# FrozenWolf-Cyber/Indic-CL-ASR

Measured on AMD Instinct MI355X. Metric: utterances/sec (15 s @16 kHz) Conformer-M RNNT-CTC+EWC train step, higher is better.
Workload: dtype bf16; 1 GPU; BASELINE configs[1]: Conformer-medium (d=256, 16L, H=640) hybrid RNNT-CTC + EWC, bs=32/GPU x 15 s, bf16 projections, freeze_encoder_till=12, 22x257 heads, fused_batch_size=4; global_batch=32, parallelism=dp1

## Files before the change

indic_cl_asr_amd/csrc/lstm.hip:

```cpp
#include <hip/hip_bf16.h>

#include <stdlib.h>

#include "ia_common.h"

namespace {

typedef __bf16 bf8 __attribute__((ext_vector_type(8)));
typedef float f4 __attribute__((ext_vector_type(4)));
typedef __attribute__((address_space(1))) unsigned gu32;

constexpr int LS_HB = 16;
constexpr int LS_THREADS = 256;
constexpr int LS_MAXB = 32;
constexpr unsigned LS_SPIN_LIMIT = 1u << 22;
constexpr int LS_STICKY_WORD = 32;

__device__ __forceinline__ float sigmoidf_(float x) { return 1.f / (1.f + __expf(-x)); }

__device__ __forceinline__ void grid_arrive(unsigned* counter) {
    asm volatile("s_waitcnt vmcnt(0)" ::: "memory");
    __syncthreads();
    if (threadIdx.x == 0) __hip_atomic_fetch_add(counter, 1u, __ATOMIC_RELAXED, __HIP_MEMORY_SCOPE_AGENT);
}
__device__ __forceinline__ void ls_store_pair(__bf16* p, float v, bool live) {
    union { __bf16 h; unsigned short u; } me;
    me.h = (__bf16)v;
    const unsigned mine = me.u;
    const unsigned other = (unsigned)__shfl_down((int)mine, 1, 64);
    if (live && !(threadIdx.x & 1))
        __hip_atomic_store((gu32*)(unsigned*)(void*)p, mine | (other << 16), __ATOMIC_RELAXED, __HIP_MEMORY_SCOPE_AGENT);
}
__device__ __forceinline__ void grid_wait(unsigned* counter, unsigned target, unsigned* status, unsigned spin_limit) {
    if (threadIdx.x == 0) {
        unsigned spins = 0;
        while (__hip_atomic_load(counter, __ATOMIC_RELAXED, __HIP_MEMORY_SCOPE_AGENT) < target) {
            __builtin_amdgcn_s_sleep(2);
            if (++spins > spin_limit) {
                __hip_atomic_store(status + 1, 1u, __ATOMIC_RELAXED, __HIP_MEMORY_SCOPE_AGENT);
                __hip_atomic_store(status + LS_STICKY_WORD, 1u, __ATOMIC_RELAXED, __HIP_MEMORY_SCOPE_AGENT);
                break;
            }
        }
        __builtin_amdgcn_fence(__ATOMIC_ACQUIRE, "agent");
        asm volatile("s_waitcnt vmcnt(0)" ::: "memory");
    }
    __syncthreads();
}

__global__ __launch_bounds__(LS_THREADS, 1) void lstm_fwd_kernel(
    const float* __restrict__ Gx,
    const __bf16* __restrict__ Whh,
    float* __restrict__ Hout,
    float* __restrict__ gates,
    float* __restrict__ Cs,
    __bf16* hx,
    unsigned* sync,
    int U, int B, int H, unsigned spin_limit) {
    extern __shared__ __attribute__((aligned(16))) unsigned char smem[];
    const int wrow = H * 2 + 16;
    unsigned char* sW = smem;
    unsigned char* sH = sW + 64 * wrow;
    float* sG = reinterpret_cast<float*>(sH + LS_MAXB * wrow);
    const int tid = threadIdx.x, lane = tid & 63, wave = tid >> 6, c = lane & 15, q4 = lane >> 4;
    const int j = blockIdx.x, nb = gridDim.x, u0 = j * LS_HB;
    const int nrt = (B + 15) / 16;
    for (int i = tid; i < 64 * (H / 8); i += LS_THREADS) {
        const int r = i / (H / 8), v = i - r * (H / 8);
        const int gate = r >> 4, ul = r & 15;
        *reinterpret_cast<uint4*>(sW + r * wrow + v * 16) =
            *reinterpret_cast<const uint4*>(Whh + (size_t)(gate * H + u0 + ul) * H + v * 8);
    }
    for (int i = tid; i < (LS_MAXB - B) * (H / 8); i += LS_THREADS) {
        const int r = B + i / (H / 8), v = i % (H / 8);
        *reinterpret_cast<uint4*>(sH + r * wrow + v * 16) = make_uint4(0, 0, 0, 0);
    }
    constexpr int EPT = (LS_MAXB * LS_HB) / LS_THREADS;
    float cst[EPT];
#pragma unroll
    for (int k = 0; k < EPT; ++k) cst[k] = 0.f;
    __syncthreads();
    float gxp[EPT][4];
#define LS_FETCH_GX(t_)                                                                                   \
    _Pragma("unroll") for (int k = 0; k < EPT; ++k) {                                                     \
        const int e_ = tid + LS_THREADS * k, b_ = e_ >> 4, ul_ = e_ & 15;                                 \
        const size_t gx_ = ((size_t)(t_) * B + (b_ < B ? b_ : B - 1)) * (4 * H) + u0 + ul_;              \
        gxp[k][0] = Gx[gx_]; gxp[k][1] = Gx[gx_ + H]; gxp[k][2] = Gx[gx_ + 2 * H]; gxp[k][3] = Gx[gx_ + 3 * H]; \
    }
    LS_FETCH_GX(0);
    for (int t = 0; t < U; ++t) {
        constexpr int NRT = LS_MAXB / 16;
        f4 acc[NRT];
#pragma unroll
        for (int rt = 0; rt < NRT; ++rt) acc[rt] = (f4){0.f, 0.f, 0.f, 0.f};
        if (t > 0) {
            grid_wait(sync, (unsigned)(nb * t), sync, spin_limit);
            const __bf16* hsrc = hx + (size_t)((t - 1) & 1) * B * H;
            for (int i = tid; i < B * (H / 8); i += LS_THREADS) {
                const int r = i / (H / 8), v = i - r * (H / 8);
                *reinterpret_cast<uint4*>(sH + r * wrow + v * 16) = *reinterpret_cast<const uint4*>(hsrc + (size_t)r * H + v * 8);
            }
            __syncthreads();
            const unsigned char* wb = sW + (wave * 16 + c) * wrow + q4 * 16;
            for (int ks = 0; ks < H / 32; ++ks) {
                const bf8 wf = *reinterpret_cast<const bf8*>(wb + ks * 64);
#pragma unroll
                for (int rt = 0; rt < NRT; ++rt)
                    if (rt < nrt) {
                        const bf8 hf = *reinterpret_cast<const bf8*>(sH + (rt * 16 + c) * wrow + q4 * 16 + ks * 64);
                        acc[rt] = __builtin_amdgcn_mfma_f32_16x16x32_bf16(hf, wf, acc[rt], 0, 0, 0);
                    }
            }
        }
#pragma unroll
        for (int rt = 0; rt < NRT; ++rt)
            if (rt < nrt)
#pragma unroll
                for (int r = 0; r < 4; ++r) sG[(wave * LS_MAXB + rt * 16 + q4 * 4 + r) * 16 + c] = acc[rt][r];
        __syncthreads();
        __bf16* hdst = hx + (size_t)(t & 1) * B * H;
        float kg[EPT][4], kh[EPT];
#pragma unroll
        for (int k = 0; k < EPT; ++k) {
            const int e = tid + LS_THREADS * k, b = e >> 4, ul = e & 15;
            if (b < B) {
                const float gi = sigmoidf_(sG[(0 * LS_MAXB + b) * 16 + ul] + gxp[k][0]);
                const float gf = sigmoidf_(sG[(1 * LS_MAXB + b) * 16 + ul] + gxp[k][1]);
                const float gg = tanhf(sG[(2 * LS_MAXB + b) * 16 + ul] + gxp[k][2]);
                const float go = sigmoidf_(sG[(3 * LS_MAXB + b) * 16 + ul] + gxp[k][3]);
                cst[k] = gf * cst[k] + gi * gg;
                const float h = go * tanhf(cst[k]);
                kg[k][0] = gi; kg[k][1] = gf; kg[k][2] = gg; kg[k][3] = go; kh[k] = h;
            } else {
                kh[k] = 0.f;
            }
            ls_store_pair(hdst + (size_t)(b < B ? b : 0) * H + u0 + ul, kh[k], b < B);
        }
        if (t + 1 < U) grid_arrive(sync);
#pragma unroll
        for (int k = 0; k < EPT; ++k) {
            const int e = tid + LS_THREADS * k, b = e >> 4, ul = e & 15;
            if (b < B) {
                const size_t gx = ((size_t)t * B + b) * (4 * H) + u0 + ul;
                const size_t ho = ((size_t)t * B + b) * H + u0 + ul;
                Hout[ho] = kh[k];
                if (gates) {
                    gates[gx] = kg[k][0]; gates[gx + H] = kg[k][1]; gates[gx + 2 * H] = kg[k][2]; gates[gx + 3 * H] = kg[k][3];
                    Cs[ho] = cst[k];
                }
            }
        }
        if (t + 1 < U) LS_FETCH_GX(t + 1);
    }
#undef LS_FETCH_GX
}

__global__ __launch_bounds__(LS_THREADS, 1) void lstm_bwd_kernel(
    const float* __restrict__ dHout,
    const float* __restrict__ gates,
    const float* __restrict__ Cs,
    const __bf16* __restrict__ WhhT,
    float* __restrict__ dG,
    __bf16* dgx,
    unsigned* sync, int U, int B, int H, unsigned spin_limit) {
    extern __shared__ __attribute__((aligned(16))) unsigned char smem[];
    const int H4 = 4 * H;
    const int wrow = H4 * 2 + 16;
    unsigned char* sW = smem;
    float* sP = reinterpret_cast<float*>(sW + LS_HB * wrow);
    const int tid = threadIdx.x, lane = tid & 63, wave = tid >> 6, c = lane & 15, q4 = lane >> 4;
    const int j = blockIdx.x, nb = gridDim.x, u0 = j * LS_HB;
    const int nrt = (B + 15) / 16;
    for (int i = tid; i < LS_HB * (H4 / 8); i += LS_THREADS) {
        const int r = i / (H4 / 8), v = i - r * (H4 / 8);
        *reinterpret_cast<uint4*>(sW + r * wrow + v * 16) = *reinterpret_cast<const uint4*>(WhhT + (size_t)(u0 + r) * H4 + v * 8);
    }
    constexpr int EPT = (LS_MAXB * LS_HB) / LS_THREADS;
    float dcc[EPT];
#pragma unroll
    for (int k = 0; k < EPT; ++k) dcc[k] = 0.f;
    __syncthreads();
    const int ksteps = H4 / 32, kper = (ksteps + 3) / 4;
    float pv[EPT][7];
#define LS_FETCH_SAVED(t_)                                                                                \
    _Pragma("unroll") for (int k = 0; k < EPT; ++k) {                                                     \
        const int e_ = tid + LS_THREADS * k, b_ = e_ >> 4, ul_ = e_ & 15;                                 \
        const int bc_ = b_ < B ? b_ : B - 1;                                                              \
        const size_t ho_ = ((size_t)(t_) * B + bc_) * H + u0 + ul_;                                       \
        const size_t gx_ = ((size_t)(t_) * B + bc_) * H4 + u0 + ul_;                                      \
        pv[k][0] = dHout[ho_]; pv[k][1] = gates[gx_]; pv[k][2] = gates[gx_ + H]; pv[k][3] = gates[gx_ + 2 * H]; \
        pv[k][4] = gates[gx_ + 3 * H]; pv[k][5] = Cs[ho_]; pv[k][6] = ((t_) > 0) ? Cs[ho_ - (size_t)B * H] : 0.f; \
    }
    LS_FETCH_SAVED(U - 1);
    for (int t = U - 1; t >= 0; --t) {
        const int phase = U - 1 - t;
        constexpr int NRT = LS_MAXB / 16;
        f4 acc[NRT];
#pragma unroll
        for (int rt = 0; rt < NRT; ++rt) acc[rt] = (f4){0.f, 0.f, 0.f, 0.f};
        if (t < U - 1) {
            grid_wait(sync, (unsigned)(nb * phase), sync, spin_limit);
            const __bf16* src = dgx + (size_t)((phase - 1) & 1) * B * H4;
            const int k0 = wave * kper, k1 = (k0 + kper < ksteps) ? (k0 + kper) : ksteps;
            for (int ks = k0; ks < k1; ++ks) {
                const bf8 wf = *reinterpret_cast<const bf8*>(sW + c * wrow + ks * 64 + q4 * 16);
#pragma unroll
                for (int rt = 0; rt < NRT; ++rt)
                    if (rt < nrt) {
                        int brow = rt * 16 + c;
                        brow = brow < B ? brow : B - 1;
                        const bf8 df = *reinterpret_cast<const bf8*>(src + (size_t)brow * H4 + ks * 32 + q4 * 8);
                        acc[rt] = __builtin_amdgcn_mfma_f32_16x16x32_bf16(df, wf, acc[rt], 0, 0, 0);
                    }
            }
        }
#pragma unroll
        for (int rt = 0; rt < NRT; ++rt)
            if (rt < nrt)
#pragma unroll
                for (int r = 0; r < 4; ++r) sP[(wave * LS_MAXB + rt * 16 + q4 * 4 + r) * 16 + c] = acc[rt][r];
        __syncthreads();
        __bf16* dst = dgx + (size_t)(phase & 1) * B * H4;
        float kd[EPT][4];
#pragma unroll
        for (int k = 0; k < EPT; ++k) {
            const int e = tid + LS_THREADS * k, b = e >> 4, ul = e & 15;
            if (b < B) {
                const float dhrec = sP[(0 * LS_MAXB + b) * 16 + ul] + sP[(1 * LS_MAXB + b) * 16 + ul] +
                                    sP[(2 * LS_MAXB + b) * 16 + ul] + sP[(3 * LS_MAXB + b) * 16 + ul];
                const float dh = pv[k][0] + dhrec;
                const float gi = pv[k][1], gf = pv[k][2], gg = pv[k][3], go = pv[k][4];
                const float ct = pv[k][5], cprev = pv[k][6];
                const float tc = tanhf(ct);
                const float dct = dh * go * (1.f - tc * tc) + dcc[k];
                const float di = dct * gg * gi * (1.f - gi);
                const float dfg = dct * cprev * gf * (1.f - gf);
                const float dgg = dct * gi * (1.f - gg * gg);
                const float dout = dh * tc * go * (1.f - go);
                dcc[k] = dct * gf;
                kd[k][0] = di; kd[k][1] = dfg; kd[k][2] = dgg; kd[k][3] = dout;
            } else {
                kd[k][0] = kd[k][1] = kd[k][2] = kd[k][3] = 0.f;
            }
            {
                __bf16* xo = dst + (size_t)(b < B ? b : 0) * H4 + u0 + ul;
#pragma unroll
                for (int gte = 0; gte < 4; ++gte) ls_store_pair(xo + (size_t)gte * H, kd[k][gte], b < B);
            }
        }
        if (t > 0) grid_arrive(sync);
#pragma unroll
        for (int k = 0; k < EPT; ++k) {
            const int e = tid + LS_THREADS * k, b = e >> 4, ul = e & 15;
            if (b < B) {
                const size_t gx = ((size_t)t * B + b) * H4 + u0 + ul;
                dG[gx] = kd[k][0]; dG[gx + H] = kd[k][1]; dG[gx + 2 * H] = kd[k][2]; dG[gx + 3 * H] = kd[k][3];
            }
        }
        if (t > 0) LS_FETCH_SAVED(t - 1);
        __syncthreads();
    }
#undef LS_FETCH_SAVED
}

}

extern "C" size_t ia_lstm_scratch_bytes(int B, int H) {
    if (B <= 0 || H <= 0) return 0;
    return 256 + ia_align_up((size_t)2 * B * 4 * H * sizeof(__bf16), 256);
}

static unsigned lstm_spin_limit() {
    const char* e = getenv("IA_LSTM_SPIN_LIMIT");
    if (e && *e) { const long v = atol(e); if (v >= 0) return (unsigned)v; }
    return LS_SPIN_LIMIT;
}

extern "C" int ia_lstm_lds_bytes(int H, int backward) {
    if (H <= 0) return 0;
    return backward ? (int)((size_t)LS_HB * (4 * H * 2 + 16) + 4 * LS_MAXB * 16 * sizeof(float))
                    : (int)((size_t)(64 + LS_MAXB) * (H * 2 + 16) + 4 * LS_MAXB * 16 * sizeof(float));
}

static int lstm_check(int U, int B, int H) {
    if (U <= 0 || B <= 0 || H <= 0) return IA_INVALID_VALUE;
    if (B > LS_MAXB || H % 32 != 0 || H % LS_HB != 0 || H / LS_HB > 256) return IA_UNSUPPORTED;
    return IA_OK;
}

extern "C" int ia_lstm_forward(const float* Gx, const void* Whh_bf16, float* Hout, float* gates, float* Cs, int U, int B,
                               int H, void* scratch, size_t scratch_bytes, ia_stream_t stream) {
    if (!Gx || !Whh_bf16 || !Hout || !scratch || (gates && !Cs)) return IA_INVALID_VALUE;
    const int rc = lstm_check(U, B, H);
    if (rc != IA_OK) return rc;
    if (scratch_bytes < ia_lstm_scratch_bytes(B, H) || !ia_is_aligned(scratch, 256) || !ia_is_aligned(Whh_bf16, 16))
        return IA_INVALID_VALUE;
    hipStream_t st = (hipStream_t)stream;
    if (hipMemsetAsync(scratch, 0, 128, st) != hipSuccess) return IA_LAUNCH_FAILED;
    const size_t lds = (size_t)(64 + LS_MAXB) * (H * 2 + 16) + 4 * LS_MAXB * 16 * sizeof(float);
    if (lds > 160 * 1024) return IA_UNSUPPORTED;
    IA_SET_MAX_LDS_ONCE((lstm_fwd_kernel), (int)lds);
    hipLaunchKernelGGL(lstm_fwd_kernel, dim3(H / LS_HB), dim3(LS_THREADS), lds, st, Gx, (const __bf16*)Whh_bf16, Hout, gates, Cs,
                       (__bf16*)((char*)scratch + 256), (unsigned*)scratch, U, B, H, lstm_spin_limit());
    IA_RETURN_IF_LAUNCH_FAILED();
    return IA_OK;
}

extern "C" int ia_lstm_backward(const float* dHout, const float* gates, const float* Cs, const void* WhhT_bf16, float* dG,
                                int U, int B, int H, void* scratch, size_t scratch_bytes, ia_stream_t stream) {
    if (!dHout || !gates || !Cs || !WhhT_bf16 || !dG || !scratch) return IA_INVALID_VALUE;
    const int rc = lstm_check(U, B, H);
    if (rc != IA_OK) return rc;
    if (scratch_bytes < ia_lstm_scratch_bytes(B, H) || !ia_is_aligned(scratch, 256) || !ia_is_aligned(WhhT_bf16, 16))
        return IA_INVALID_VALUE;
    hipStream_t st = (hipStream_t)stream;
    if (hipMemsetAsync(scratch, 0, 128, st) != hipSuccess) return IA_LAUNCH_FAILED;
    const size_t lds = (size_t)LS_HB * (4 * H * 2 + 16) + 4 * LS_MAXB * 16 * sizeof(float);
    if (lds > 160 * 1024) return IA_UNSUPPORTED;
    IA_SET_MAX_LDS_ONCE((lstm_bwd_kernel), (int)lds);
    hipLaunchKernelGGL(lstm_bwd_kernel, dim3(H / LS_HB), dim3(LS_THREADS), lds, st, dHout, gates, Cs, (const __bf16*)WhhT_bf16, dG,
                       (__bf16*)((char*)scratch + 256), (unsigned*)scratch, U, B, H, lstm_spin_limit());
    IA_RETURN_IF_LAUNCH_FAILED();
    return IA_OK;
}
```

indic_cl_asr_amd/csrc/dwconv.hip:

```cpp
#include <hip/hip_bf16.h>

#include <cstdint>
#include <cstdlib>

#include "ia_common.h"
#include "indicasr.h"
#include "partials.h"

namespace {

constexpr int DW_TT = 16;
constexpr int DW_TB = 4 * DW_TT;

template <int KMAX>
__device__ __forceinline__ void load_taps(float (&wt)[KMAX], const float* __restrict__ w, int c, int ksz, int flip) {
    const int off = (KMAX - 1) / 2 - (ksz - 1) / 2;
#pragma unroll
    for (int jj = 0; jj < KMAX; ++jj) {
        const int j = jj - off;
        wt[jj] = (j >= 0 && j < ksz) ? w[c * ksz + (flip ? ksz - 1 - j : j)] : 0.f;
    }
}

template <int KMAX, int GLU>
// ... 129 lines not shown
    if (wv == 0 && cok) {
        float* row = part + (size_t)blockIdx.x * (KMAX + 1) * d;
#pragma unroll
        for (int jj = 0; jj < KMAX; ++jj)
            row[(size_t)jj * d + c] = (acc[jj] + red[0][jj][lane]) + (red[1][jj][lane] + red[2][jj][lane]);
        row[(size_t)KMAX * d + c] = (sb + red[0][KMAX][lane]) + (red[1][KMAX][lane] + red[2][KMAX][lane]);
    }
}

__global__ __launch_bounds__(256) void dwconv_wgrad_finish_kernel(const float* __restrict__ part, int G, int d, int kmax, int ksz,
                                                                  float* __restrict__ dw, float* __restrict__ db) {
    __shared__ float red[8][32];
    const int o = threadIdx.x & 31, sl = threadIdx.x >> 5;
    const int idx = blockIdx.x * 32 + o, total = (kmax + 1) * d;
    float a0 = 0.f, a1 = 0.f;
    if (idx < total) {
        int g = sl;
        for (; g + 8 < G; g += 16) { a0 += part[(size_t)g * total + idx]; a1 += part[(size_t)(g + 8) * total + idx]; }
        for (; g < G; g += 8) a0 += part[(size_t)g * total + idx];
    }
    red[sl][o] = a0 + a1;
    __syncthreads();
    if (sl != 0 || idx >= total) return;
    const float s = ((red[0][o] + red[1][o]) + (red[2][o] + red[3][o])) + ((red[4][o] + red[5][o]) + (red[6][o] + red[7][o]));
    const int jj = idx / d, c = idx - jj * d;
    if (jj == kmax) {
        if (db) db[c] = s;
    } else {
        const int j = jj - ((kmax - 1) / 2 - (ksz - 1) / 2);
        if (j >= 0 && j < ksz) dw[c * ksz + j] = s;
    }
}

inline int kmax_for(int ksz) { return ksz <= 9 ? 9 : (ksz <= 15 ? 15 : 31); }

inline int wgrad_splits(int B, int T, int d) {
    const int cg = (d + 63) / 64;
    int ns = (768 + B * cg - 1) / (B * cg);
    const int cap = (T + DW_TB - 1) / DW_TB;
    if (ns > cap) ns = cap;
    return ns < 1 ? 1 : ns;
}

inline bool dw_shape_ok(int d, int ksz) { return d > 0 && d <= 4096 && ksz >= 1 && ksz <= 31 && (ksz & 1) == 1; }

}

extern "C" int64_t ia_dwconv_scratch_elems(int B, int T, int d, int ksz) {
    if (B <= 0 || T <= 0 || !dw_shape_ok(d, ksz)) return 0;
    const int64_t fwd = (int64_t)B * ((T + DW_TB - 1) / DW_TB) * 2 * d;
    const int64_t wg = (int64_t)B * wgrad_splits(B, T, d) * (kmax_for(ksz) + 1) * d;
    return fwd > wg ? fwd : wg;
}

extern "C" int ia_glu_dwconv(const void* x2, const int64_t* lens, int B, int T, int d, int ksz, const float* w,
                             const float* bias, float* z, float* bn_sum, float* bn_sumsq, float* scratch,
                             ia_stream_t stream) {
    if (!x2 || !lens || !w || !bias || !z || !bn_sum || !bn_sumsq || !scratch || B <= 0 || T <= 0) return IA_INVALID_VALUE;
    if (!dw_shape_ok(d, ksz)) return IA_UNSUPPORTED;
    hipStream_t st = (hipStream_t)stream;
    const dim3 grid(B * ((T + DW_TB - 1) / DW_TB), (d + 63) / 64), blk(256);
#define IA_DWF(K) hipLaunchKernelGGL((dwconv_fwd_kernel<K, 1>), grid, blk, 0, st, x2, lens, B, T, d, ksz, w, bias, 0, z, scratch, (long long*)nullptr)
    switch (kmax_for(ksz)) {
        case 9: IA_DWF(9); break;
        case 15: IA_DWF(15); break;
        default: IA_DWF(31); break;
    }
#undef IA_DWF
    IA_RETURN_IF_LAUNCH_FAILED();
    ia_partials_finish(scratch, (int)grid.x, 2 * d, d, bn_sum, bn_sumsq, st);
    IA_RETURN_IF_LAUNCH_FAILED();
    return IA_OK;
}

extern "C" int ia_glu_dwconv_fixed(const void* x2, const int64_t* lens, int B, int T, int d, int ksz, const float* w,
                                   const float* bias, float* z, long long* bn_sums_fixed, ia_stream_t stream) {
    if (!x2 || !lens || !w || !bias || !z || !bn_sums_fixed || B <= 0 || T <= 0) return IA_INVALID_VALUE;
    if (!dw_shape_ok(d, ksz)) return IA_UNSUPPORTED;
    hipStream_t st = (hipStream_t)stream;
    const dim3 grid(B * ((T + DW_TB - 1) / DW_TB), (d + 63) / 64), blk(256);
#define IA_DWF(K) hipLaunchKernelGGL((dwconv_fwd_kernel<K, 1>), grid, blk, 0, st, x2, lens, B, T, d, ksz, w, bias, 0, z, (float*)nullptr, bn_sums_fixed)
    switch (kmax_for(ksz)) {
        case 9: IA_DWF(9); break;
        case 15: IA_DWF(15); break;
        default: IA_DWF(31); break;
    }
#undef IA_DWF
    IA_RETURN_IF_LAUNCH_FAILED();
    return IA_OK;
}

extern "C" int ia_dwconv_gated_fixed(const void* g, const int64_t* lens, int B, int T, int d, int ksz, const float* w,
                                     const float* bias, float* z, long long* bn_sums_fixed, ia_stream_t stream) {
    if (!g || !lens || !w || !bias || !z || !bn_sums_fixed || B <= 0 || T <= 0) return IA_INVALID_VALUE;
    if (!dw_shape_ok(d, ksz)) return IA_UNSUPPORTED;
    hipStream_t st = (hipStream_t)stream;
    const dim3 grid(B * ((T + DW_TB - 1) / DW_TB), (d + 63) / 64), blk(256);
#define IA_DWF(K) hipLaunchKernelGGL((dwconv_fwd_kernel<K, 2>), grid, blk, 0, st, g, lens, B, T, d, ksz, w, bias, 0, z, (float*)nullptr, bn_sums_fixed)
    switch (kmax_for(ksz)) {
        case 9: IA_DWF(9); break;
        case 15: IA_DWF(15); break;
        default: IA_DWF(31); break;
    }
#undef IA_DWF
    IA_RETURN_IF_LAUNCH_FAILED();
    return IA_OK;
}

extern "C" int ia_dwconv_time(const float* x, int B, int T, int d, int ksz, const float* w, const float* bias, int flip,
                              float* y, ia_stream_t stream) {
    if (!x || !w || !y || B <= 0 || T <= 0) return IA_INVALID_VALUE;
    if (!dw_shape_ok(d, ksz)) return IA_UNSUPPORTED;
    hipStream_t st = (hipStream_t)stream;
    const dim3 grid(B * ((T + DW_TB - 1) / DW_TB), (d + 63) / 64), blk(256);
#define IA_DWF(K) hipLaunchKernelGGL((dwconv_fwd_kernel<K, 0>), grid, blk, 0, st, (const void*)x, (const int64_t*)nullptr, B, T, d, ksz, w, bias, flip, y, (float*)nullptr, (long long*)nullptr)
    switch (kmax_for(ksz)) {
        case 9: IA_DWF(9); break;
        case 15: IA_DWF(15); break;
        default: IA_DWF(31); break;
    }
#undef IA_DWF
    IA_RETURN_IF_LAUNCH_FAILED();
    return IA_OK;
}

extern "C" int ia_dwconv_time_wgrad(const float* x, const float* dy, int B, int T, int d, int ksz, float* dw, float* db,
                                    float* scratch, ia_stream_t stream) {
    if (!x || !dy || !dw || !scratch || B <= 0 || T <= 0) return IA_INVALID_VALUE;
    if (!dw_shape_ok(d, ksz)) return IA_UNSUPPORTED;
    hipStream_t st = (hipStream_t)stream;
    const int ns = wgrad_splits(B, T, d), kmax = kmax_for(ksz);
    const dim3 grid(B * ns, (d + 63) / 64), blk(256);
#define IA_DWG(K) hipLaunchKernelGGL((dwconv_wgrad_kernel<K, false>), grid, blk, 0, st, x, dy, B, T, d, ns, scratch, (const __bf16*)nullptr, (const int64_t*)nullptr)
    switch (kmax) {
        case 9: IA_DWG(9); break;
        case 15: IA_DWG(15); break;
        default: IA_DWG(31); break;
    }
#undef IA_DWG
    IA_RETURN_IF_LAUNCH_FAILED();
    hipLaunchKernelGGL(dwconv_wgrad_finish_kernel, dim3(((kmax + 1) * d + 31) / 32), dim3(256), 0, st, scratch, (int)grid.x, d,
                       kmax, ksz, dw, db);
    IA_RETURN_IF_LAUNCH_FAILED();
    return IA_OK;
}

extern "C" int ia_dwconv_glu_bwd(const float* dz, const void* c2, const int64_t* lens, int B, int T, int d, int ksz, const float* w,
                                 void* dc2, ia_stream_t stream) {
    if (!dz || !c2 || !lens || !w || !dc2 || B <= 0 || T <= 0) return IA_INVALID_VALUE;
    if (!dw_shape_ok(d, ksz)) return IA_UNSUPPORTED;
    hipStream_t st = (hipStream_t)stream;
    const dim3 grid(B * ((T + DW_TB - 1) / DW_TB), (d + 63) / 64), blk(256);
#define IA_DWF(K) hipLaunchKernelGGL((dwconv_fwd_kernel<K, 3>), grid, blk, 0, st, (const void*)dz, lens, B, T, d, ksz, w, (const float*)nullptr, 1, (float*)nullptr, (float*)nullptr, (long long*)nullptr, (const __bf16*)c2, (__bf16*)dc2)
    switch (kmax_for(ksz)) {
        case 9: IA_DWF(9); break;
        case 15: IA_DWF(15); break;
        default: IA_DWF(31); break;
    }
#undef IA_DWF
    IA_RETURN_IF_LAUNCH_FAILED();
    return IA_OK;
}

extern "C" int ia_dwconv_glu_wgrad(const void* c2, const int64_t* lens, const float* dy, int B, int T, int d, int ksz, float* dw,
                                   float* db, float* scratch, ia_stream_t stream) {
    if (!c2 || !lens || !dy || !dw || !scratch || B <= 0 || T <= 0) return IA_INVALID_VALUE;
    if (!dw_shape_ok(d, ksz)) return IA_UNSUPPORTED;
    hipStream_t st = (hipStream_t)stream;
    const int ns = wgrad_splits(B, T, d), kmax = kmax_for(ksz);
    const dim3 grid(B * ns, (d + 63) / 64), blk(256);
#define IA_DWG(K) hipLaunchKernelGGL((dwconv_wgrad_kernel<K, true>), grid, blk, 0, st, (const float*)nullptr, dy, B, T, d, ns, scratch, (const __bf16*)c2, lens)
    switch (kmax) {
        case 9: IA_DWG(9); break;
        case 15: IA_DWG(15); break;
        default: IA_DWG(31); break;
    }
#undef IA_DWG
    IA_RETURN_IF_LAUNCH_FAILED();
    hipLaunchKernelGGL(dwconv_wgrad_finish_kernel, dim3(((kmax + 1) * d + 31) / 32), dim3(256), 0, st, scratch, (int)grid.x, d,
                       kmax, ksz, dw, db);
    IA_RETURN_IF_LAUNCH_FAILED();
    return IA_OK;
}
```

Before: 3779 utterances/s.

## Keep LSTM recurrent weights resident in registers instead of LDS for H=640/320

Adds templated LSTM forward and backward kernels that preload each wave's slice of the recurrent weight matrix into bf8 registers once. Each timestep's MFMA loop then reads only h or dgates from LDS or global memory, not the weights, so per-step LDS traffic drops and the LDS footprint shrinks. The K loops are fully unrolled with a compile-time step count, and the FMA ordering is pinned explicitly. The cost is much higher register pressure, and the launch bounds now ask for two blocks per CU. The path is limited to H of 640 or 320 and can be turned off with an environment variable.

Measured after the change: 3788 utterances/s, median of 5. Within noise of the previous version (+0.2%).

```diff
diff --git a/indic_cl_asr_amd/csrc/lstm.hip b/indic_cl_asr_amd/csrc/lstm.hip
--- a/indic_cl_asr_amd/csrc/lstm.hip
+++ b/indic_cl_asr_amd/csrc/lstm.hip
@@ -17,6 +17,7 @@
 constexpr int LS_STICKY_WORD = 32;
 
 __device__ __forceinline__ float sigmoidf_(float x) { return 1.f / (1.f + __expf(-x)); }
+
 
 __device__ __forceinline__ void grid_arrive(unsigned* counter) {
     asm volatile("s_waitcnt vmcnt(0)" ::: "memory");
@@ -48,7 +49,37 @@
     __syncthreads();
 }
 
-__global__ __launch_bounds__(LS_THREADS, 1) void lstm_fwd_kernel(
+__host__ __device__ constexpr size_t ls_fwd_lds(int H, bool wreg) {
+    return (size_t)((wreg ? 0 : 64) + LS_MAXB) * (H * 2 + 16) + 4 * LS_MAXB * LS_HB * sizeof(float);
+}
+__host__ __device__ constexpr size_t ls_bwd_lds(int H, bool wreg) {
+    return (wreg ? 0 : (size_t)LS_HB * (4 * H * 2 + 16)) + 4 * LS_MAXB * LS_HB * sizeof(float);
+}
+
+template <int KS, int NR>
+__device__ __forceinline__ void ls_fwd_dot(f4 (&acc)[LS_MAXB / 16], const bf8 (&wf)[KS], const unsigned char* hb, int wrow) {
+#pragma unroll
+    for (int ks = 0; ks < KS; ++ks)
+#pragma unroll
+        for (int rt = 0; rt < NR; ++rt) {
+            const bf8 hf = *reinterpret_cast<const bf8*>(hb + rt * 16 * wrow + ks * 64);
+            acc[rt] = __builtin_amdgcn_mfma_f32_16x16x32_bf16(hf, wf[ks], acc[rt], 0, 0, 0);
+        }
+}
+template <int KS, int NR>
+__device__ __forceinline__ void ls_bwd_dot(f4 (&acc)[LS_MAXB / 16], const bf8 (&wf)[KS], const __bf16* const (&drow)[LS_MAXB / 16],
+                                           int kofs) {
+#pragma unroll
+    for (int i = 0; i < KS; ++i)
+#pragma unroll
+        for (int rt = 0; rt < NR; ++rt) {
+            const bf8 df = *reinterpret_cast<const bf8*>(drow[rt] + kofs + i * 32);
+            acc[rt] = __builtin_amdgcn_mfma_f32_16x16x32_bf16(df, wf[i], acc[rt], 0, 0, 0);
+        }
+}
+
+template <int KS>
+__global__ __launch_bounds__(LS_THREADS, KS ? 2 : 1) void lstm_fwd_kernel(
     const float* __restrict__ Gx,
     const __bf16* __restrict__ Whh,
     float* __restrict__ Hout,
@@ -56,20 +87,28 @@
     float* __restrict__ Cs,
     __bf16* hx,
     unsigned* sync,
-    int U, int B, int H, unsigned spin_limit) {
+    int U, int B, int Hrt, unsigned spin_limit) {
     extern __shared__ __attribute__((aligned(16))) unsigned char smem[];
+    const int H = KS ? KS * 32 : Hrt;
     const int wrow = H * 2 + 16;
     unsigned char* sW = smem;
-    unsigned char* sH = sW + 64 * wrow;
+    unsigned char* sH = sW + (KS ? 0 : 64) * wrow;
     float* sG = reinterpret_cast<float*>(sH + LS_MAXB * wrow);
     const int tid = threadIdx.x, lane = tid & 63, wave = tid >> 6, c = lane & 15, q4 = lane >> 4;
     const int j = blockIdx.x, nb = gridDim.x, u0 = j * LS_HB;
     const int nrt = (B + 15) / 16;
-    for (int i = tid; i < 64 * (H / 8); i += LS_THREADS) {
-        const int r = i / (H / 8), v = i - r * (H / 8);
-        const int gate = r >> 4, ul = r & 15;
-        *reinterpret_cast<uint4*>(sW + r * wrow + v * 16) =
-            *reinterpret_cast<const uint4*>(Whh + (size_t)(gate * H + u0 + ul) * H + v * 8);
+    bf8 wf[KS ? KS : 1];
+    if constexpr (KS > 0) {
+        const __bf16* wg = Whh + (size_t)(wave * H + u0 + c) * H + q4 * 8;
+#pragma unroll
+        for (int ks = 0; ks < KS; ++ks) wf[ks] = *reinterpret_cast<const bf8*>(wg + ks * 32);
+    } else {
+        for (int i = tid; i < 64 * (H / 8); i += LS_THREADS) {
+            const int r = i / (H / 8), v = i - r * (H / 8);
+            const int gate = r >> 4, ul = r & 15;
+            *reinterpret_cast<uint4*>(sW + r * wrow + v * 16) =
+                *reinterpret_cast<const uint4*>(Whh + (size_t)(gate * H + u0 + ul) * H + v * 8);
+        }
     }
     for (int i = tid; i < (LS_MAXB - B) * (H / 8); i += LS_THREADS) {
         const int r = B + i / (H / 8), v = i % (H / 8);
@@ -101,15 +140,21 @@
                 *reinterpret_cast<uint4*>(sH + r * wrow + v * 16) = *reinterpret_cast<const uint4*>(hsrc + (size_t)r * H + v * 8);
             }
             __syncthreads();
-            const unsigned char* wb = sW + (wave * 16 + c) * wrow + q4 * 16;
-            for (int ks = 0; ks < H / 32; ++ks) {
-                const bf8 wf = *reinterpret_cast<const bf8*>(wb + ks * 64);
-#pragma unroll
-                for (int rt = 0; rt < NRT; ++rt)
-                    if (rt < nrt) {
-                        const bf8 hf = *reinterpret_cast<const bf8*>(sH + (rt * 16 + c) * wrow + q4 * 16 + ks * 64);
-                        acc[rt] = __builtin_amdgcn_mfma_f32_16x16x32_bf16(hf, wf, acc[rt], 0, 0, 0);
-                    }
+            const unsigned char* hb = sH + c * wrow + q4 * 16;
+            if constexpr (KS > 0) {
+                if (nrt == NRT) ls_fwd_dot<KS, NRT>(acc, wf, hb, wrow);
+                else ls_fwd_dot<KS, 1>(acc, wf, hb, wrow);
+            } else {
+                const unsigned char* wb = sW + (wave * 16 + c) * wrow + q4 * 16;
+                for (int ks = 0; ks < H / 32; ++ks) {
+                    const bf8 wl = *reinterpret_cast<const bf8*>(wb + ks * 64);
+#pragma unroll
+                    for (int rt = 0; rt < NRT; ++rt)
+                        if (rt < nrt) {
+                            const bf8 hf = *reinterpret_cast<const bf8*>(hb + rt * 16 * wrow + ks * 64);
+                            acc[rt] = __builtin_amdgcn_mfma_f32_16x16x32_bf16(hf, wl, acc[rt], 0, 0, 0);
+                        }
+                }
             }
         }
 #pragma unroll
@@ -122,13 +167,14 @@
         float kg[EPT][4], kh[EPT];
 #pragma unroll
         for (int k = 0; k < EPT; ++k) {
+#pragma clang fp contract(off)
             const int e = tid + LS_THREADS * k, b = e >> 4, ul = e & 15;
             if (b < B) {
                 const float gi = sigmoidf_(sG[(0 * LS_MAXB + b) * 16 + ul] + gxp[k][0]);
                 const float gf = sigmoidf_(sG[(1 * LS_MAXB + b) * 16 + ul] + gxp[k][1]);
                 const float gg = tanhf(sG[(2 * LS_MAXB + b) * 16 + ul] + gxp[k][2]);
                 const float go = sigmoidf_(sG[(3 * LS_MAXB + b) * 16 + ul] + gxp[k][3]);
-                cst[k] = gf * cst[k] + gi * gg;
+                cst[k] = __builtin_fmaf(gi, gg, gf * cst[k]);
                 const float h = go * tanhf(cst[k]);
                 kg[k][0] = gi; kg[k][1] = gf; kg[k][2] = gg; kg[k][3] = go; kh[k] = h;
             } else {
@@ -155,32 +201,42 @@
 #undef LS_FETCH_GX
 }
 
-__global__ __launch_bounds__(LS_THREADS, 1) void lstm_bwd_kernel(
+template <int KS>
+__global__ __launch_bounds__(LS_THREADS, KS ? 2 : 1) void lstm_bwd_kernel(
     const float* __restrict__ dHout,
     const float* __restrict__ gates,
     const float* __restrict__ Cs,
     const __bf16* __restrict__ WhhT,
     float* __restrict__ dG,
     __bf16* dgx,
-    unsigned* sync, int U, int B, int H, unsigned spin_limit) {
+    unsigned* sync, int U, int B, int Hrt, unsigned spin_limit) {
     extern __shared__ __attribute__((aligned(16))) unsigned char smem[];
+    const int H = KS ? KS * 32 : Hrt;
     const int H4 = 4 * H;
     const int wrow = H4 * 2 + 16;
     unsigned char* sW = smem;
-    float* sP = reinterpret_cast<float*>(sW + LS_HB * wrow);
+    float* sP = reinterpret_cast<float*>(sW + (KS ? 0 : LS_HB) * wrow);
     const int tid = threadIdx.x, lane = tid & 63, wave = tid >> 6, c = lane & 15, q4 = lane >> 4;
     const int j = blockIdx.x, nb = gridDim.x, u0 = j * LS_HB;
     const int nrt = (B + 15) / 16;
-    for (int i = tid; i < LS_HB * (H4 / 8); i += LS_THREADS) {
-        const int r = i / (H4 / 8), v = i - r * (H4 / 8);
-        *reinterpret_cast<uint4*>(sW + r * wrow + v * 16) = *reinterpret_cast<const uint4*>(WhhT + (size_t)(u0 + r) * H4 + v * 8);
+    const int ksteps = H4 / 32, kper = (ksteps + 3) / 4;
+    const int k0 = wave * kper, k1 = (k0 + kper < ksteps) ? (k0 + kper) : ksteps;
+    bf8 wf[KS ? KS : 1];
+    if constexpr (KS > 0) {
+        const __bf16* wg = WhhT + (size_t)(u0 + c) * H4 + k0 * 32 + q4 * 8;
+#pragma unroll
+        for (int i = 0; i < KS; ++i) wf[i] = *reinterpret_cast<const bf8*>(wg + i * 32);
+    } else {
+        for (int i = tid; i < LS_HB * (H4 / 8); i += LS_THREADS) {
+            const int r = i / (H4 / 8), v = i - r * (H4 / 8);
+            *reinterpret_cast<uint4*>(sW + r * wrow + v * 16) = *reinterpret_cast<const uint4*>(WhhT + (size_t)(u0 + r) * H4 + v * 8);
+        }
     }
     constexpr int EPT = (LS_MAXB * LS_HB) / LS_THREADS;
     float dcc[EPT];
 #pragma unroll
     for (int k = 0; k < EPT; ++k) dcc[k] = 0.f;
     __syncthreads();
-    const int ksteps = H4 / 32, kper = (ksteps + 3) / 4;
     float pv[EPT][7];
 #define LS_FETCH_SAVED(t_)                                                                                \
     _Pragma("unroll") for (int k = 0; k < EPT; ++k) {                                                     \
@@ -201,17 +257,25 @@
         if (t < U - 1) {
             grid_wait(sync, (unsigned)(nb * phase), sync, spin_limit);
             const __bf16* src = dgx + (size_t)((phase - 1) & 1) * B * H4;
-            const int k0 = wave * kper, k1 = (k0 + kper < ksteps) ? (k0 + kper) : ksteps;
-            for (int ks = k0; ks < k1; ++ks) {
-                const bf8 wf = *reinterpret_cast<const bf8*>(sW + c * wrow + ks * 64 + q4 * 16);
-#pragma unroll
-                for (int rt = 0; rt < NRT; ++rt)
-                    if (rt < nrt) {
-                        int brow = rt * 16 + c;
-                        brow = brow < B ? brow : B - 1;
-                        const bf8 df = *reinterpret_cast<const bf8*>(src + (size_t)brow * H4 + ks * 32 + q4 * 8);
-                        acc[rt] = __builtin_amdgcn_mfma_f32_16x16x32_bf16(df, wf, acc[rt], 0, 0, 0);
-                    }
+            const __bf16* drow[NRT];
+#pragma unroll
+            for (int rt = 0; rt < NRT; ++rt) {
+                const int brow = rt * 16 + c;
+                drow[rt] = src + (size_t)(brow < B ? brow : B - 1) * H4 + q4 * 8;
+            }
+            if constexpr (KS > 0) {
+                if (nrt == NRT) ls_bwd_dot<KS, NRT>(acc, wf, drow, k0 * 32);
+                else ls_bwd_dot<KS, 1>(acc, wf, drow, k0 * 32);
+            } else {
+                for (int ks = k0; ks < k1; ++ks) {
+                    const bf8 wl = *reinterpret_cast<const bf8*>(sW + c * wrow + ks * 64 + q4 * 16);
+#pragma unroll
+                    for (int rt = 0; rt < NRT; ++rt)
+                        if (rt < nrt) {
+                            const bf8 df = *reinterpret_cast<const bf8*>(drow[rt] + ks * 32);
+                            acc[rt] = __builtin_amdgcn_mfma_f32_16x16x32_bf16(df, wl, acc[rt], 0, 0, 0);
+                        }
+                }
             }
         }
 #pragma unroll
@@ -224,6 +288,7 @@
         float kd[EPT][4];
 #pragma unroll
         for (int k = 0; k < EPT; ++k) {
+#pragma clang fp contract(off)
             const int e = tid + LS_THREADS * k, b = e >> 4, ul = e & 15;
             if (b < B) {
                 const float dhrec = sP[(0 * LS_MAXB + b) * 16 + ul] + sP[(1 * LS_MAXB + b) * 16 + ul] +
@@ -232,7 +297,7 @@
                 const float gi = pv[k][1], gf = pv[k][2], gg = pv[k][3], go = pv[k][4];
                 const float ct = pv[k][5], cprev = pv[k][6];
                 const float tc = tanhf(ct);
-                const float dct = dh * go * (1.f - tc * tc) + dcc[k];
+                const float dct = __builtin_fmaf(dh * go, 1.f - tc * tc, dcc[k]);
                 const float di = dct * gg * gi * (1.f - gi);
                 const float dfg = dct * cprev * gf * (1.f - gf);
                 const float dgg = dct * gi * (1.f - gg * gg);
@@ -276,15 +341,46 @@
     return LS_SPIN_LIMIT;
 }
 
+static int lstm_wreg_ksteps(int H) {
+    if (H != 640 && H != 320) return 0;
+    const char* e = getenv("IA_LSTM_WREG");
+    if (e && e[0] == '0' && !e[1]) return 0;
+    return H / 32;
+}
+
 extern "C" int ia_lstm_lds_bytes(int H, int backward) {
     if (H <= 0) return 0;
-    return backward ? (int)((size_t)LS_HB * (4 * H * 2 + 16) + 4 * LS_MAXB * 16 * sizeof(float))
-                    : (int)((size_t)(64 + LS_MAXB) * (H * 2 + 16) + 4 * LS_MAXB * 16 * sizeof(float));
+    const bool wreg = lstm_wreg_ksteps(H) > 0;
+    return (int)(backward ? ls_bwd_lds(H, wreg) : ls_fwd_lds(H, wreg));
 }
 
 static int lstm_check(int U, int B, int H) {
     if (U <= 0 || B <= 0 || H <= 0) return IA_INVALID_VALUE;
     if (B > LS_MAXB || H % 32 != 0 || H % LS_HB != 0 || H / LS_HB > 256) return IA_UNSUPPORTED;
+    return IA_OK;
+}
+
+template <int KS>
+static int lstm_launch_fwd(const float* Gx, const __bf16* Whh, float* Hout, float* gates, float* Cs, int U, int B, int H,
+                           void* scratch, hipStream_t st) {
+    const size_t lds = ls_fwd_lds(H, KS > 0);
+    if (lds > 160 * 1024) return IA_UNSUPPORTED;
+    IA_SET_MAX_LDS_ONCE((lstm_fwd_kernel<KS>), (int)lds);
+    hipLaunchKernelGGL((lstm_fwd_kernel<KS>), dim3(H / LS_HB), dim3(LS_THREADS), lds, st, Gx, Whh, Hout, gates, Cs,
+                       (__bf16*)((char*)scratch + 256), (unsigned*)scratch, U, B, H, lstm_spin_limit());
+    IA_RETURN_IF_LAUNCH_FAILED();
+    return IA_OK;
+}
+
+template <int KS>
+static int lstm_launch_bwd(const float* dHout, const float* gates, const float* Cs, const __bf16* WhhT, float* dG, int U, int B,
+                           int H, void* scratch, hipStream_t st) {
+    const size_t lds = ls_bwd_lds(H, KS > 0);
+    if (lds > 160 * 1024) return IA_UNSUPPORTED;
+    IA_SET_MAX_LDS_ONCE((lstm_bwd_kernel<KS>), (int)lds);
+    hipLaunchKernelGGL((lstm_bwd_kernel<KS>), dim3(H / LS_HB), dim3(LS_THREADS), lds, st, dHout, gates, Cs, WhhT, dG,
+                       (__bf16*)((char*)scratch + 256), (unsigned*)scratch, U, B, H, lstm_spin_limit());
+    IA_RETURN_IF_LAUNCH_FAILED();
     return IA_OK;
 }
 
@@ -297,13 +393,12 @@
         return IA_INVALID_VALUE;
     hipStream_t st = (hipStream_t)stream;
     if (hipMemsetAsync(scratch, 0, 128, st) != hipSuccess) return IA_LAUNCH_FAILED;
-    const size_t lds = (size_t)(64 + LS_MAXB) * (H * 2 + 16) + 4 * LS_MAXB * 16 * sizeof(float);
-    if (lds > 160 * 1024) return IA_UNSUPPORTED;
-    IA_SET_MAX_LDS_ONCE((lstm_fwd_kernel), (int)lds);
-    hipLaunchKernelGGL(lstm_fwd_kernel, dim3(H / LS_HB), dim3(LS_THREADS), lds, st, Gx, (const __bf16*)Whh_bf16, Hout, gates, Cs,
-                       (__bf16*)((char*)scratch + 256), (unsigned*)scratch, U, B, H, lstm_spin_limit());
-    IA_RETURN_IF_LAUNCH_FAILED();
-    return IA_OK;
+    const __bf16* W = (const __bf16*)Whh_bf16;
+    switch (lstm_wreg_ksteps(H)) {
+        case 20: return lstm_launch_fwd<20>(Gx, W, Hout, gates, Cs, U, B, H, scratch, st);
+        case 10: return lstm_launch_fwd<10>(Gx, W, Hout, gates, Cs, U, B, H, scratch, st);
+        default: return lstm_launch_fwd<0>(Gx, W, Hout, gates, Cs, U, B, H, scratch, st);
+    }
 }
 
 extern "C" int ia_lstm_backward(const float* dHout, const float* gates, const float* Cs, const void* WhhT_bf16, float* dG,
@@ -315,11 +410,10 @@
         return IA_INVALID_VALUE;
     hipStream_t st = (hipStream_t)stream;
     if (hipMemsetAsync(scratch, 0, 128, st) != hipSuccess) return IA_LAUNCH_FAILED;
-    const size_t lds = (size_t)LS_HB * (4 * H * 2 + 16) + 4 * LS_MAXB * 16 * sizeof(float);
-    if (lds > 160 * 1024) return IA_UNSUPPORTED;
-    IA_SET_MAX_LDS_ONCE((lstm_bwd_kernel), (int)lds);
-    hipLaunchKernelGGL(lstm_bwd_kernel, dim3(H / LS_HB), dim3(LS_THREADS), lds, st, dHout, gates, Cs, (const __bf16*)WhhT_bf16, dG,
-                       (__bf16*)((char*)scratch + 256), (unsigned*)scratch, U, B, H, lstm_spin_limit());
-    IA_RETURN_IF_LAUNCH_FAILED();
-    return IA_OK;
-}
+    const __bf16* W = (const __bf16*)WhhT_bf16;
+    switch (lstm_wreg_ksteps(H)) {
+        case 20: return lstm_launch_bwd<20>(dHout, gates, Cs, W, dG, U, B, H, scratch, st);
+        case 10: return lstm_launch_bwd<10>(dHout, gates, Cs, W, dG, U, B, H, scratch, st);
+        default: return lstm_launch_bwd<0>(dHout, gates, Cs, W, dG, U, B, H, scratch, st);
+    }
+}
```

## Stage depthwise-conv input windows and taps in LDS with vectorized loads

Applied to the files above, without the earlier changes.

Adds LDS-tiled variants of the depthwise conv forward, GLU backward and weight-gradient kernels. Each block now loads its time window (with halo), the per-channel taps and the c2 rows into shared memory using 16-byte vector loads, then reads them from LDS, instead of each thread loading rows directly from global memory. The goal is to cut redundant global reads and improve coalescing for the conformer conv module. The old kernels stay reachable through the IA_DWCONV_V1 environment variable; the new path adds LDS use and extra barriers, which may lower occupancy.

Result: slower. 3701 utterances/s before, 3607 utterances/s after (-2.5%).

```diff
diff --git a/indic_cl_asr_amd/csrc/dwconv.hip b/indic_cl_asr_amd/csrc/dwconv.hip
--- a/indic_cl_asr_amd/csrc/dwconv.hip
+++ b/indic_cl_asr_amd/csrc/dwconv.hip
@@ -185,6 +185,268 @@
     }
 }
 
+
+constexpr int DW_SRC_F32 = 0, DW_SRC_GLU = 1, DW_SRC_BF16 = 2;
+
+__device__ __forceinline__ bool dw_aligned16(const void* p) { return (reinterpret_cast<uintptr_t>(p) & 15) == 0; }
+
+__device__ __forceinline__ void stage_taps(float* __restrict__ wl, const float* __restrict__ w, int c0, int d, int ksz) {
+    const int nch = d - c0 < 64 ? d - c0 : 64, n = nch * ksz;
+    const float* src = w + (size_t)c0 * ksz;
+    int done = 0;
+    if (dw_aligned16(src)) {
+        const int n4 = n >> 2;
+        for (int i = threadIdx.x; i < n4; i += 256) reinterpret_cast<float4*>(wl)[i] = reinterpret_cast<const float4*>(src)[i];
+        done = n4 << 2;
+    }
+    for (int i = done + threadIdx.x; i < n; i += 256) wl[i] = src[i];
+}
+
+template <int KMAX>
+__device__ __forceinline__ void read_taps(float (&wt)[KMAX], const float* __restrict__ wl, int lc, int ksz, int flip) {
+    const int off = (KMAX - 1) / 2 - (ksz - 1) / 2;
+#pragma unroll
+    for (int jj = 0; jj < KMAX; ++jj) {
+        const int j = jj - off;
+        wt[jj] = (j >= 0 && j < ksz) ? wl[lc * ksz + (flip ? ksz - 1 - j : j)] : 0.f;
+    }
+}
+
+__device__ __forceinline__ void bf16x8_to_f32(const uint4& u, float (&f)[8]) {
+    const __bf16* h = reinterpret_cast<const __bf16*>(&u);
+#pragma unroll
+    for (int i = 0; i < 8; ++i) f[i] = (float)h[i];
+}
+
+template <int R, int SRC>
+__device__ __forceinline__ void stage_rows(float* __restrict__ tile, const void* __restrict__ src, size_t row0, int T, int tfirst,
+                                           int tmax, int d, int c0) {
+    const int tid = threadIdx.x;
+    if constexpr (SRC == DW_SRC_F32) {
+        const float* x = reinterpret_cast<const float*>(src);
+        if ((d & 3) == 0 && dw_aligned16(x)) {
+            const int q = tid & 15, c = c0 + 4 * q;
+            const bool cin = c < d;
+#pragma unroll
+            for (int p = 0; p < (R + 15) / 16; ++p) {
+                int r = p * 16 + (tid >> 4);
+                r = r < R ? r : R - 1;
+                const int t = tfirst + r, tt = t < 0 ? 0 : (t >= T ? T - 1 : t);
+                float4 v = *reinterpret_cast<const float4*>(x + (row0 + tt) * d + (cin ? c : 0));
+                if (!(cin && t >= 0 && t < tmax)) v = make_float4(0.f, 0.f, 0.f, 0.f);
+                *reinterpret_cast<float4*>(tile + r * 64 + 4 * q) = v;
+            }
+            return;
+        }
+    } else {
+        const __bf16* x = reinterpret_cast<const __bf16*>(src);
+        if ((d & 7) == 0 && dw_aligned16(x)) {
+            const int q = tid & 7, c = c0 + 8 * q;
+            const bool cin = c < d;
+            const size_t ld = SRC == DW_SRC_GLU ? 2 * (size_t)d : (size_t)d;
+#pragma unroll
+            for (int p = 0; p < (R + 31) / 32; ++p) {
+                int r = p * 32 + (tid >> 3);
+                r = r < R ? r : R - 1;
+                const int t = tfirst + r, tt = t < 0 ? 0 : (t >= T ? T - 1 : t);
+                const __bf16* pr = x + (row0 + tt) * ld + (cin ? c : 0);
+                float v[8];
+                bf16x8_to_f32(*reinterpret_cast<const uint4*>(pr), v);
+                if constexpr (SRC == DW_SRC_GLU) {
+                    float g[8];
+                    bf16x8_to_f32(*reinterpret_cast<const uint4*>(pr + d), g);
+#pragma unroll
+                    for (int i = 0; i < 8; ++i) v[i] = v[i] * ia_sigmoid_fast(g[i]);
+                }
+                const bool ok = cin && t >= 0 && t < tmax;
+#pragma unroll
+                for (int i = 0; i < 8; ++i) v[i] = ok ? v[i] : 0.f;
+                float4* o = reinterpret_cast<float4*>(tile + r * 64 + 8 * q);
+                o[0] = make_float4(v[0], v[1], v[2], v[3]);
+                o[1] = make_float4(v[4], v[5], v[6], v[7]);
+            }
+            return;
+        }
+    }
+    for (int idx = tid; idx < R * 64; idx += 256) {
+        const int r = idx >> 6, c = c0 + (idx & 63);
+        const int t = tfirst + r, tt = t < 0 ? 0 : (t >= T ? T - 1 : t);
+        const int cc = c < d ? c : d - 1;
+        float v;
+        if constexpr (SRC == DW_SRC_GLU) {
+            const __bf16* p = reinterpret_cast<const __bf16*>(src) + (row0 + tt) * (2 * (size_t)d);
+            const float a = (float)p[cc], gate = (float)p[d + cc];
+            v = a * ia_sigmoid_fast(gate);
+        } else if constexpr (SRC == DW_SRC_BF16) {
+            v = (float)reinterpret_cast<const __bf16*>(src)[(row0 + tt) * d + cc];
+        } else {
+            v = reinterpret_cast<const float*>(src)[(row0 + tt) * d + cc];
+        }
+        tile[idx] = (c < d && t >= 0 && t < tmax) ? v : 0.f;
+    }
+}
+
+__device__ __forceinline__ void stage_c2(__bf16* __restrict__ cl, const __bf16* __restrict__ c2, size_t row0, int T, int tfirst, int d,
+                                         int c0) {
+    const int tid = threadIdx.x;
+    if ((d & 7) == 0 && dw_aligned16(c2)) {
+        const int q = tid & 7, h = (tid >> 3) & 1, c = c0 + 8 * q;
+        uint4 v[DW_TB / 16];
+#pragma unroll
+        for (int p = 0; p < DW_TB / 16; ++p) {
+            const int t = tfirst + p * 16 + (tid >> 4), tt = t >= T ? T - 1 : t;
+            v[p] = *reinterpret_cast<const uint4*>(c2 + (row0 + tt) * (2 * (size_t)d) + (size_t)h * d + (c < d ? c : 0));
+        }
+#pragma unroll
+        for (int p = 0; p < DW_TB / 16; ++p)
+            *reinterpret_cast<uint4*>(cl + (p * 16 + (tid >> 4)) * 128 + h * 64 + 8 * q) = v[p];
+        return;
+    }
+    for (int idx = tid; idx < DW_TB * 128; idx += 256) {
+        const int r = idx >> 7, h = (idx >> 6) & 1, c = c0 + (idx & 63);
+        const int t = tfirst + r, tt = t >= T ? T - 1 : t;
+        cl[idx] = c2[(row0 + tt) * (2 * (size_t)d) + (size_t)h * d + (c < d ? c : d - 1)];
+    }
+}
+
+template <int KMAX, int GLU>
+__global__ __launch_bounds__(256) void dwconv_fwd_lds_kernel(const void* __restrict__ xin, const int64_t* __restrict__ lens, int B,
+                                                             int T, int d, int ksz, const float* __restrict__ w,
+                                                             const float* __restrict__ bias, int flip, float* __restrict__ y,
+                                                             float* __restrict__ part, long long* __restrict__ acc,
+                                                             const __bf16* __restrict__ c2 = nullptr, __bf16* __restrict__ dc2 = nullptr) {
+    constexpr int HM = (KMAX - 1) / 2, WIN = DW_TT + KMAX - 1, R = DW_TB + KMAX - 1;
+    static_assert(GLU >= 1 && GLU <= 3, "GLU = 0 stays on dwconv_fwd_kernel (see the file header)");
+    static_assert(R * 64 * sizeof(float) >= DW_TB * 128 * sizeof(__bf16), "the c2 rows reuse the window tile");
+    __shared__ __attribute__((aligned(16))) float tile[R * 64];
+    __shared__ __attribute__((aligned(16))) float wl[64 * KMAX];
+    const int lane = threadIdx.x & 63, wv = threadIdx.x >> 6;
+    const int ntb = (T + DW_TB - 1) / DW_TB;
+    const int b = blockIdx.x / ntb, tb = (blockIdx.x - b * ntb) * DW_TB, t0 = tb + wv * DW_TT;
+    const int c0 = blockIdx.y * 64, c = c0 + lane;
+    const bool cok = c < d;
+    const int cc = cok ? c : d - 1;
+    const int len = (int)lens[b];
+    const int tmax = (GLU == 3 || len >= T) ? T : len;
+    stage_taps(wl, w, c0, d, ksz);
+    stage_rows<R, GLU == 1 ? DW_SRC_GLU : (GLU == 2 ? DW_SRC_BF16 : DW_SRC_F32)>(tile, xin, (size_t)b * T, T, tb - HM, tmax, d, c0);
+    __syncthreads();
+    float wt[KMAX];
+    read_taps<KMAX>(wt, wl, cc - c0, ksz, flip);
+    float win[WIN];
+#pragma unroll
+    for (int r = 0; r < WIN; ++r) win[r] = tile[(wv * DW_TT + r) * 64 + lane];
+    __bf16* cl = reinterpret_cast<__bf16*>(tile);
+    if (GLU == 3) {
+        __syncthreads();
+        stage_c2(cl, c2, (size_t)b * T, T, tb, d, c0);
+        __syncthreads();
+    }
+    const float bb = bias ? bias[cc] : 0.f;
+    float s = 0.f, s2 = 0.f;
+#pragma unroll
+    for (int i = 0; i < DW_TT; ++i) {
+        float acc = bb;
+#pragma unroll
+        for (int jj = 0; jj < KMAX; ++jj) acc = __builtin_fmaf(wt[jj], win[i + jj], acc);
+        const int t = t0 + i;
+        if (t < T && cok) {
+            if (GLU == 3) {
+                const size_t row = (size_t)b * T + t;
+                const float av = (float)cl[(wv * DW_TT + i) * 128 + lane], gv = (float)cl[(wv * DW_TT + i) * 128 + 64 + lane];
+                const float sg = ia_sigmoid_fast(gv);
+                const float dg = (t < len) ? acc : 0.f;
+                dc2[row * 2 * d + c] = (__bf16)(dg * sg);
+                dc2[row * 2 * d + d + c] = (__bf16)(dg * av * sg * (1.f - sg));
+            } else {
+                y[((size_t)b * T + t) * d + c] = acc;
+                {
+#pragma clang fp contract(off)
+                    s += acc; s2 += acc * acc;
+                }
+            }
+        }
+    }
+    if (GLU == 1 || GLU == 2) {
+        __shared__ float red[4][2][64];
+        red[wv][0][lane] = s; red[wv][1][lane] = s2;
+        __syncthreads();
+        if (wv == 0 && cok) {
+            const float t1 = (red[0][0][lane] + red[1][0][lane]) + (red[2][0][lane] + red[3][0][lane]);
+            const float t2 = (red[0][1][lane] + red[1][1][lane]) + (red[2][1][lane] + red[3][1][lane]);
+            if (acc) {
+                long long* mine = acc + (size_t)(blockIdx.x & (IA_BN_ACC_COPIES - 1)) * 2 * d;
+                atomicAdd(reinterpret_cast<unsigned long long*>(mine + c), (unsigned long long)__float2ll_rn(t1 * 16777216.f));
+                atomicAdd(reinterpret_cast<unsigned long long*>(mine + d + c), (unsigned long long)__float2ll_rn(t2 * 16777216.f));
+            } else {
+                part[(size_t)blockIdx.x * 2 * d + c] = t1;
+                part[(size_t)blockIdx.x * 2 * d + d + c] = t2;
+            }
+        }
+    }
+}
+
+template <int KMAX>
+__global__ __launch_bounds__(256) void dwconv_wgrad_lds_kernel(const float* __restrict__ dy, int B, int T, int d, int nsplit,
+                                                               float* __restrict__ part, const __bf16* __restrict__ c2,
+                                                               const int64_t* __restrict__ lens) {
+    constexpr int HM = (KMAX - 1) / 2, WIN = DW_TT + KMAX - 1, R = DW_TB + KMAX - 1;
+    constexpr int NSTAGE = (R + DW_TB) * 64, NRED = 3 * (KMAX + 1) * 64;
+    __shared__ __attribute__((aligned(16))) float sm[NSTAGE > NRED ? NSTAGE : NRED];
+    float* tile = sm;
+    float* gl = sm + R * 64;
+    const int lane = threadIdx.x & 63, wv = threadIdx.x >> 6;
+    const int b = blockIdx.x / nsplit, sp = blockIdx.x - b * nsplit;
+    const int per = (((T + nsplit - 1) / nsplit + DW_TT - 1) / DW_TT) * DW_TT;
+    const int ts = sp * per, te = (ts + per < T) ? ts + per : T;
+    const int c0 = blockIdx.y * 64, c = c0 + lane;
+    const bool cok = c < d;
+    float acc[KMAX];
+#pragma unroll
+    for (int jj = 0; jj < KMAX; ++jj) acc[jj] = 0.f;
+    float sb = 0.f;
+    const int len = (int)lens[b], tlen = len < T ? len : T;
+    for (int tb = ts; tb < te; tb += DW_TB) {
+        if (tb != ts) __syncthreads();
+        stage_rows<R, DW_SRC_GLU>(tile, c2, (size_t)b * T, T, tb - HM, tlen, d, c0);
+        stage_rows<DW_TB, DW_SRC_F32>(gl, dy, (size_t)b * T, T, tb, te, d, c0);
+        __syncthreads();
+        if (tb + wv * DW_TT < te) {
+            float g[DW_TT], win[WIN];
+#pragma unroll
+            for (int i = 0; i < DW_TT; ++i) g[i] = gl[(wv * DW_TT + i) * 64 + lane];
+#pragma unroll
+            for (int r = 0; r < WIN; ++r) win[r] = tile[(wv * DW_TT + r) * 64 + lane];
+#pragma unroll
+            for (int i = 0; i < DW_TT; ++i) {
+                sb += g[i];
+#pragma unroll
+                for (int jj = 0; jj < KMAX; ++jj) acc[jj] = __builtin_fmaf(g[i], win[i + jj], acc[jj]);
+            }
+        }
+    }
+    __syncthreads();
+    float* red = sm;
+    if (wv > 0) {
+#pragma unroll
+        for (int jj = 0; jj < KMAX; ++jj) red[((wv - 1) * (KMAX + 1) + jj) * 64 + lane] = acc[jj];
+        red[((wv - 1) * (KMAX + 1) + KMAX) * 64 + lane] = sb;
+    }
+    __syncthreads();
+    if (wv == 0 && cok) {
+        float* row = part + (size_t)blockIdx.x * (KMAX + 1) * d;
+#pragma unroll
+        for (int jj = 0; jj < KMAX; ++jj)
+            row[(size_t)jj * d + c] = (acc[jj] + red[jj * 64 + lane]) + (red[((KMAX + 1) + jj) * 64 + lane] + red[(2 * (KMAX + 1) + jj) * 64 + lane]);
+        row[(size_t)KMAX * d + c] = (sb + red[KMAX * 64 + lane]) + (red[((KMAX + 1) + KMAX) * 64 + lane] + red[(2 * (KMAX + 1) + KMAX) * 64 + lane]);
+    }
+}
+
+inline bool dw_v1() {
+    const char* e = getenv("IA_DWCONV_V1");
+    return e && e[0] == '1';
+}
+
 inline int kmax_for(int ksz) { return ksz <= 9 ? 9 : (ksz <= 15 ? 15 : 31); }
 
 inline int wgrad_splits(int B, int T, int d) {
@@ -199,6 +461,12 @@
 
 }
 
+#define IA_DW_FWD(K, G, ...)                                                                                  \
+    do {                                                                                                      \
+        if (v1) hipLaunchKernelGGL((dwconv_fwd_kernel<K, G>), grid, blk, 0, st, __VA_ARGS__);                 \
+        else hipLaunchKernelGGL((dwconv_fwd_lds_kernel<K, G>), grid, blk, 0, st, __VA_ARGS__);                \
+    } while (0)
+
 extern "C" int64_t ia_dwconv_scratch_elems(int B, int T, int d, int ksz) {
     if (B <= 0 || T <= 0 || !dw_shape_ok(d, ksz)) return 0;
     const int64_t fwd = (int64_t)B * ((T + DW_TB - 1) / DW_TB) * 2 * d;
@@ -212,8 +480,9 @@
     if (!x2 || !lens || !w || !bias || !z || !bn_sum || !bn_sumsq || !scratch || B <= 0 || T <= 0) return IA_INVALID_VALUE;
     if (!dw_shape_ok(d, ksz)) return IA_UNSUPPORTED;
     hipStream_t st = (hipStream_t)stream;
+    const bool v1 = dw_v1();
     const dim3 grid(B * ((T + DW_TB - 1) / DW_TB), (d + 63) / 64), blk(256);
-#define IA_DWF(K) hipLaunchKernelGGL((dwconv_fwd_kernel<K, 1>), grid, blk, 0, st, x2, lens, B, T, d, ksz, w, bias, 0, z, scratch, (long long*)nullptr)
+#define IA_DWF(K) IA_DW_FWD(K, 1, x2, lens, B, T, d, ksz, w, bias, 0, z, scratch, (long long*)nullptr)
     switch (kmax_for(ksz)) {
         case 9: IA_DWF(9); break;
         case 15: IA_DWF(15); break;
@@ -231,8 +500,9 @@
     if (!x2 || !lens || !w || !bias || !z || !bn_sums_fixed || B <= 0 || T <= 0) return IA_INVALID_VALUE;
     if (!dw_shape_ok(d, ksz)) return IA_UNSUPPORTED;
     hipStream_t st = (hipStream_t)stream;
+    const bool v1 = dw_v1();
     const dim3 grid(B * ((T + DW_TB - 1) / DW_TB), (d + 63) / 64), blk(256);
-#define IA_DWF(K) hipLaunchKernelGGL((dwconv_fwd_kernel<K, 1>), grid, blk, 0, st, x2, lens, B, T, d, ksz, w, bias, 0, z, (float*)nullptr, bn_sums_fixed)
+#define IA_DWF(K) IA_DW_FWD(K, 1, x2, lens, B, T, d, ksz, w, bias, 0, z, (float*)nullptr, bn_sums_fixed)
     switch (kmax_for(ksz)) {
         case 9: IA_DWF(9); break;
         case 15: IA_DWF(15); break;
@@ -248,8 +518,9 @@
     if (!g || !lens || !w || !bias || !z || !bn_sums_fixed || B <= 0 || T <= 0) return IA_INVALID_VALUE;
     if (!dw_shape_ok(d, ksz)) return IA_UNSUPPORTED;
     hipStream_t st = (hipStream_t)stream;
+    const bool v1 = dw_v1();
     const dim3 grid(B * ((T + DW_TB - 1) / DW_TB), (d + 63) / 64), blk(256);
-#define IA_DWF(K) hipLaunchKernelGGL((dwconv_fwd_kernel<K, 2>), grid, blk, 0, st, g, lens, B, T, d, ksz, w, bias, 0, z, (float*)nullptr, bn_sums_fixed)
+#define IA_DWF(K) IA_DW_FWD(K, 2, g, lens, B, T, d, ksz, w, bias, 0, z, (float*)nullptr, bn_sums_fixed)
     switch (kmax_for(ksz)) {
         case 9: IA_DWF(9); break;
         case 15: IA_DWF(15); break;
@@ -303,8 +574,9 @@
     if (!dz || !c2 || !lens || !w || !dc2 || B <= 0 || T <= 0) return IA_INVALID_VALUE;
     if (!dw_shape_ok(d, ksz)) return IA_UNSUPPORTED;
     hipStream_t st = (hipStream_t)stream;
+    const bool v1 = dw_v1();
     const dim3 grid(B * ((T + DW_TB - 1) / DW_TB), (d + 63) / 64), blk(256);
-#define IA_DWF(K) hipLaunchKernelGGL((dwconv_fwd_kernel<K, 3>), grid, blk, 0, st, (const void*)dz, lens, B, T, d, ksz, w, (const float*)nullptr, 1, (float*)nullptr, (float*)nullptr, (long long*)nullptr, (const __bf16*)c2, (__bf16*)dc2)
+#define IA_DWF(K) IA_DW_FWD(K, 3, (const void*)dz, lens, B, T, d, ksz, w, (const float*)nullptr, 1, (float*)nullptr, (float*)nullptr, (long long*)nullptr, (const __bf16*)c2, (__bf16*)dc2)
     switch (kmax_for(ksz)) {
         case 9: IA_DWF(9); break;
         case 15: IA_DWF(15); break;
@@ -320,9 +592,14 @@
     if (!c2 || !lens || !dy || !dw || !scratch || B <= 0 || T <= 0) return IA_INVALID_VALUE;
     if (!dw_shape_ok(d, ksz)) return IA_UNSUPPORTED;
     hipStream_t st = (hipStream_t)stream;
+    const bool v1 = dw_v1();
     const int ns = wgrad_splits(B, T, d), kmax = kmax_for(ksz);
     const dim3 grid(B * ns, (d + 63) / 64), blk(256);
-#define IA_DWG(K) hipLaunchKernelGGL((dwconv_wgrad_kernel<K, true>), grid, blk, 0, st, (const float*)nullptr, dy, B, T, d, ns, scratch, (const __bf16*)c2, lens)
+#define IA_DWG(K)                                                                                                                \
+    do {                                                                                                                         \
+        if (v1) hipLaunchKernelGGL((dwconv_wgrad_kernel<K, true>), grid, blk, 0, st, (const float*)nullptr, dy, B, T, d, ns, scratch, (const __bf16*)c2, lens); \
+        else hipLaunchKernelGGL((dwconv_wgrad_lds_kernel<K>), grid, blk, 0, st, dy, B, T, d, ns, scratch, (const __bf16*)c2, lens); \
+    } while (0)
     switch (kmax) {
         case 9: IA_DWG(9); break;
         case 15: IA_DWG(15); break;
```
